# jsourati/nn-active-learning

Measured on AMD Instinct MI355X. Metric: patches/sec Fisher-scored (32^3, 2-class), higher is better.
Workload: dtype f32 (fp32 operands split into 16-bit pieces on the 16-bit MFMA, fp32 accumulate: fp16 pairs - 22-23 bits kept per operand, three products - in the conv under the head (forward + backward), in dec1's forward launch and in the other backward launches; bf16 triples - all 24 bits, exact, six products -

## Files before the change

nn-active-learning_amd/csrc/alq_internal.h:

```cpp
#pragma once
#include <hip/hip_runtime.h>

#include <cstdint>
#include <cstdio>
#include <memory>
#include <string>
#include <vector>

#include "alq.h"

namespace alq {

void set_error(const char *fmt, ...);

#define ALQ_HIP(expr)                                                                     \
    do {                                                                                  \
        hipError_t e_ = (expr);                                                           \
        if (e_ != hipSuccess) {                                                           \
            ::alq::set_error("%s:%d: %s -> %s", __FILE__, __LINE__, #expr,               \
                             hipGetErrorString(e_));                                      \
            return ALQ_EHIP;                                                              \
        }                                                                                 \
    } while (0)

// ... 190 lines not shown
    int mask_split = 0;
    long long mask_delta = 0;
    const unsigned char *mask_bits = nullptr;
    unsigned char *sign_out = nullptr;
    const unsigned *in_bits = nullptr;
    const float *in_vec = nullptr;
    float in_vec_amax = 0.f;
    const unsigned *in_vec16 = nullptr;
    unsigned *out_amax = nullptr;
    int amax_from = 0;
    const unsigned *in_amax = nullptr, *in_amax2 = nullptr;
    float in_bound = 0.f;
    const float *fc_W = nullptr;
    long long fc_F = 0;
    float *fc_part = nullptr;
    unsigned *fc_bits = nullptr;
    unsigned *flip_cnt = nullptr, *flip_list = nullptr;
    int flip_cap = 0;
    float flip_l1 = 0.f;
    bool flip_bias_nonzero = false;
};

extern unsigned long long *g_igemm2_dbg;
constexpr int ALQ_NKNOBS = 9;
extern int g_dbg_knobs[ALQ_NKNOBS];
extern int g_dcp_last_form;
extern int g_no_f16x2;
extern int g_no_fixed;
extern int g_no_xcd_order;
int igemm2_build_plan(const IgemmPlan &p1, Igemm2Plan *p2);
void igemm2_pack_weights(Igemm2Plan *p2, const std::vector<float> &Bmat);
int igemm2_launch(alq_ctx *ctx, const Igemm2Plan &plan, const View &in, const View &out, const float *bias,
                  int relu, int accumulate, int N, int prof_cls, const Igemm2Fuse *fuse);

struct Igemm3Plan {
    bool ok = false;
    bool wres = false;
    int NTW = 1;
    int wgs_per_cu = 1;
    size_t lds_bytes = 0;
    std::vector<unsigned short> h_W;
    void *d_W = nullptr;
    std::vector<unsigned short> h_W16;
    void *d_W16 = nullptr;
    int w16_exp = 0;
};
int igemm3_build_plan(const Igemm2Plan &p2, Igemm3Plan *p3);
void igemm3_pack_weights(const Igemm2Plan &p2, Igemm3Plan *p3, const std::vector<float> &Bmat);
void igemm3_pack_weights_f16(const Igemm2Plan &p2, Igemm3Plan *p3, const std::vector<float> &Bmat);
// ... 363 lines not shown
```

nn-active-learning_amd/csrc/igemm2.hip:

```cpp
#include "alq_internal.h"

#include <algorithm>
#include <cmath>
#include <cstring>

namespace alq {

typedef float f32x4 __attribute__((ext_vector_type(4)));
typedef float f32x2 __attribute__((ext_vector_type(2)));

#ifdef ALQ_STAMPS
#define STAMP(var) asm volatile("s_memtime %0\n\ts_waitcnt lgkmcnt(0)" : "=s"(var)::"memory")
#define PHASE_END(idx)                         \
    do {                                       \
        unsigned long long t_now_;             \
        STAMP(t_now_);                         \
        ph[idx] += t_now_ - t_last;            \
        t_last = t_now_;                       \
    } while (0)
#else
#define PHASE_END(idx) do {} while (0)
#endif

constexpr int I2_CBP = 12;
// ... 461 lines not shown
}

void igemm2_pack_weights(Igemm2Plan *p2, const std::vector<float> &Bmat) {
    const Igemm2Args &a = p2->a;
    const int NTW = p2->NTW, Ci = a.Ci, Co = a.Co;
    p2->h_W.assign((size_t)a.nchunks * a.ntaps * NTW * 128, 0.f);
    for (int ch = 0; ch < a.nchunks; ++ch)
        for (int tp = 0; tp < a.ntaps; ++tp)
            for (int nt = 0; nt < NTW; ++nt)
                for (int lane = 0; lane < 64; ++lane)
                    for (int s = 0; s < 2; ++s) {
                        const int c = ch * 8 + 2 * (lane >> 4) + s;
                        const int co = nt * 16 + (lane & 15);
                        if (co < Co)
                            p2->h_W[((((size_t)ch * a.ntaps + tp) * NTW + nt) * 64 + lane) * 2 + s] =
                                Bmat[((size_t)tp * Ci + c) * Co + co];
                    }
}

unsigned long long *g_igemm2_dbg = nullptr;
int g_no_f16x2 = 0;
int g_no_xcd_order = 0;
int g_no_fixed = 0;
int g_dbg_knobs[ALQ_NKNOBS] = {0, 0, 0, 0, 0, 0, 0, 0, 0};

template <int NTW, bool WRES, int GEO, bool SUMS>
static int launch2_s(alq_ctx *ctx, const Igemm2Plan &plan, const Igemm2Args &a, unsigned grid) {
    auto kfn = igemm2_kernel<NTW, WRES, GEO, SUMS>;
    if (plan.lds_bytes > 64 * 1024)
        ALQ_HIP(hipFuncSetAttribute(reinterpret_cast<const void *>(kfn), hipFuncAttributeMaxDynamicSharedMemorySize,
                                    (int)plan.lds_bytes));
    hipLaunchKernelGGL(kfn, dim3(grid), dim3(256), plan.lds_bytes, ctx->stream, a);
    ALQ_HIP(hipGetLastError());
    return ALQ_OK;
}

template <int NTW, bool WRES, int GEO>
static int launch2_t(alq_ctx *ctx, const Igemm2Plan &plan, const Igemm2Args &a, unsigned grid) {
    return (a.osumA || a.osumB) ? launch2_s<NTW, WRES, GEO, true>(ctx, plan, a, grid)
                                : launch2_s<NTW, WRES, GEO, false>(ctx, plan, a, grid);
}

int igemm2_launch(alq_ctx *ctx, const Igemm2Plan &plan, const View &in, const View &out, const float *bias, int relu,
                  int accumulate, int N, int prof_cls, const Igemm2Fuse *fuse) {
    Igemm2Args a = plan.a;
    ALQ_REQUIRE(in.C == a.Ci && in.D == a.ID && in.H == a.IH && in.W == a.IW, ALQ_EINVAL,
                "igemm2: input view does not match plan");
// ... 53 lines not shown
```

nn-active-learning_amd/csrc/kernels.hip:

```cpp
#include "alq_internal.h"

namespace alq {

typedef float f32x4 __attribute__((ext_vector_type(4)));
typedef float f32x2 __attribute__((ext_vector_type(2)));

constexpr int BOX_SLAB = 1024;

__device__ inline double wave_sum(double v) {
#pragma unroll
    for (int o = 32; o > 0; o >>= 1) v += __shfl_xor(v, o, 64);
    return v;
}
__device__ inline float wave_sumf(float v) {
#pragma unroll
    for (int o = 32; o > 0; o >>= 1) v += __shfl_xor(v, o, 64);
    return v;
}
__device__ inline double block_sum256(double v, double *sh ) {
    v = wave_sum(v);
    if ((threadIdx.x & 63) == 0) sh[threadIdx.x >> 6] = v;
    __syncthreads();
    double r = 0;
    if (threadIdx.x == 0) r = sh[0] + sh[1] + sh[2] + sh[3];
// ... 830 lines not shown
                                P.x += r[ex]; P.y += r[1 + ex]; P.z += r[2 + ex]; P.w += r[3 + ex];
                            }
                        }
                    }
#pragma unroll
                    for (int q = 0; q + 1 < KZ; ++q) s[q] = s[q + 1];
                    s[KZ - 1] = P;
                    if (pp >= KZ - 1) {
                        f32x4 box = s[0];
#pragma unroll
                        for (int q = 1; q < KZ; ++q) { box.x += s[q].x; box.y += s[q].y; box.z += s[q].z; box.w += s[q].w; }
                        const f32x4 dd = d[pp - (KZ - 1)];
                        acc += (double)dd.x * ((double)box.x + 1.0) + (double)dd.y * ((double)box.y + 1.0) +
                               (double)dd.z * ((double)box.z + 1.0) + (double)dd.w * ((double)box.w + 1.0);
                    }
                }
            }
        }
    }
    const double tot_s = block_sum256(acc, sh);
    if (threadIdx.x == 0) Spart[n * nslab_max + slab] = tot_s;
}

static size_t boxdot_tile_bytes(int zs, int H, int W, const int k[3]) {
    return (size_t)(zs + k[0] - 1) * (H + k[1] - 1) * (W + k[2] - 1) * sizeof(float);
}
static int boxdot_zs(int D, int H, int W, const int k[3]) {
    int zs = 4096 / (H * W);
    if (zs < 1) zs = 1;
    if (zs > D) zs = D;
    while (zs > 1 && boxdot_tile_bytes(zs, H, W, k) > 48 * 1024) --zs;
    return zs;
}
static size_t boxdot_lds_bytes(int D, int H, int W, const int k[3]) {
    return boxdot_tile_bytes(boxdot_zs(D, H, W, k), H, W, k);
}
static bool boxdot_use_lds(int D, int H, int W, const int k[3]) {
    return (long long)D * H * W >= 512 && boxdot_lds_bytes(D, H, W, k) <= 48 * 1024;
}

int boxdot_slabs(long long vox) { return (int)((vox + BOX_SLAB - 1) / BOX_SLAB); }
int boxdot_conv_slabs(int D, int H, int W, const int k[3]) {
    if (boxdot_use_lds(D, H, W, k)) { const int zs = boxdot_zs(D, H, W, k); return (D + zs - 1) / zs; }
    return boxdot_slabs((long long)D * H * W);
}

int k_boxdot_conv(alq_ctx *ctx, const float *dsum, const float *asum, const float *asum2, int D, int H, int W,
                  const int k[3], const int lo[3], int N, double *Spart, int nslab_max) {
    ProfScope ps(ctx, PROF_REDUCE, 0);
    if (boxdot_use_lds(D, H, W, k)) {
        const int zs = boxdot_zs(D, H, W, k);
        const bool al16 = (((uintptr_t)dsum | (uintptr_t)asum | (uintptr_t)asum2) & 15) == 0;
#define ALQ_BOXCOL(KZ, KY, KX)                                                                                        \
    if (k[0] == KZ && k[1] == KY && k[2] == KX && (W & 3) == 0 && al16) {                                              \
        hipLaunchKernelGGL((boxdot_conv_col_kernel<KZ, KY, KX>), dim3((D + zs - 1) / zs, N), dim3(256),               \
                           boxdot_lds_bytes(D, H, W, k), ctx->stream, dsum, asum, asum2, D, H, W, lo[0], lo[1], lo[2], \
                           zs, Spart, nslab_max);                                                                      \
        ALQ_LAUNCH_CHECK();                                                                                            \
        return ALQ_OK;                                                                                                 \
    }
        ALQ_BOXCOL(3, 3, 3)
        ALQ_BOXCOL(1, 3, 3)
        ALQ_BOXCOL(1, 5, 5)
#undef ALQ_BOXCOL
        hipLaunchKernelGGL(boxdot_conv_lds_kernel, dim3((D + zs - 1) / zs, N), dim3(256), boxdot_lds_bytes(D, H, W, k),
                           ctx->stream, dsum, asum, asum2, D, H, W, k[0], k[1], k[2], lo[0], lo[1], lo[2], zs, Spart,
                           nslab_max);
        ALQ_LAUNCH_CHECK();
        return ALQ_OK;
    }
    hipLaunchKernelGGL(boxdot_conv_kernel, dim3(boxdot_slabs((long long)D * H * W), N), dim3(256), 0, ctx->stream,
                       dsum, asum, asum2, D, H, W, k[0], k[1], k[2], lo[0], lo[1], lo[2], Spart, nslab_max);
    ALQ_LAUNCH_CHECK();
    return ALQ_OK;
}
// ... 40 lines not shown
                if (uz < 0 || qz >= ID) continue;
#pragma unroll
                for (int iy = 0; iy < (K + S - 1) / S; ++iy) {
                    const int ty = (py + ly) % S + iy * S, uy = py + ly - ty, qy = uy / S;
                    if (ty >= K || uy < 0 || qy >= IH) continue;
                    const float *rowp = tile + (qz * IH + qy) * IW;
#pragma unroll
                    for (int j = 0; j < 4; ++j)
#pragma unroll
                        for (int ix = 0; ix < (K + S - 1) / S; ++ix) {
                            const int tx = (px + j + lx) % S + ix * S, ux = px + j + lx - tx, qx = ux / S;
                            if (tx < K && ux >= 0 && qx < IW) box[j] += rowp[qx];
                        }
                }
            }
            acc += (double)d.x * ((double)box[0] + 1.0) + (double)d.y * ((double)box[1] + 1.0) +
                   (double)d.z * ((double)box[2] + 1.0) + (double)d.w * ((double)box[3] + 1.0);
        }
    }
    const double tot = block_sum256(acc, sh);
    if (threadIdx.x == 0) Spart[n * nslab_max + slab] = tot;
}

static bool boxdot_convT_out_ok(int ID, int IH, int IW, const int k[3], const int s[3]) {
    const long long ivox = (long long)ID * IH * IW;
    const bool shape = k[1] == 3 && k[2] == 3 && s[1] == 2 && s[2] == 2 &&
                       ((k[0] == 3 && s[0] == 2) || (k[0] == 1 && s[0] == 1 && ID == 1));
    return shape && ivox % 4 == 0 && ivox * 4 <= 48 * 1024;
}
static int boxdot_convT_zs(int ID, int IH, int IW, const int s[3]) {
    int zs = 4096 / (IH * s[1] * IW * s[2]);
    if (zs < 1) zs = 1;
    if (zs > ID * s[0]) zs = ID * s[0];
    return zs;
}
int boxdot_convT_slabs(int ID, int IH, int IW, const int k[3], const int s[3]) {
    if (boxdot_convT_out_ok(ID, IH, IW, k, s)) { const int zs = boxdot_convT_zs(ID, IH, IW, s); return (ID * s[0] + zs - 1) / zs; }
    return boxdot_slabs((long long)ID * IH * IW);
}

int k_boxdot_convT(alq_ctx *ctx, const float *dsum, const float *asum, const float *asum2, int ID, int IH, int IW,
                   const int k[3], const int s[3], const int lo[3], int N, double *Spart, int nslab_max) {
    ProfScope ps(ctx, PROF_REDUCE, 0);
    if (boxdot_convT_out_ok(ID, IH, IW, k, s)) {
        const int zs = boxdot_convT_zs(ID, IH, IW, s);
        hipLaunchKernelGGL((boxdot_convT_out_kernel<3, 2>), dim3((ID * s[0] + zs - 1) / zs, N), dim3(256),
                           (size_t)ID * IH * IW * sizeof(float), ctx->stream, dsum, asum, asum2, ID, IH, IW, k[0], lo[0],
                           lo[1], lo[2], zs, Spart, nslab_max);
        ALQ_LAUNCH_CHECK();
        return ALQ_OK;
    }
    hipLaunchKernelGGL(boxdot_convT_kernel, dim3(boxdot_slabs((long long)ID * IH * IW), N), dim3(256), 0,
                       ctx->stream, dsum, asum, asum2, ID, IH, IW, k[0], k[1], k[2], s[0], s[1], s[2], lo[0], lo[1], lo[2],
                       Spart, nslab_max);
    ALQ_LAUNCH_CHECK();
    return ALQ_OK;
}

constexpr int FC_SLICE = 8192;
int fc_small_slices(int64_t F) { return (int)((F + FC_SLICE - 1) / FC_SLICE); }

template <int NOUT, bool BITS>
__global__ __launch_bounds__(256) void fc_small_fwd_kernel(const float *act, long long F, const float *Wp,
                                                           float *partials, int nslices, unsigned *maskbits) {
    __shared__ double sh[4];
    const int slice = blockIdx.x;
    const long long n = blockIdx.y;
    const long long f0 = (long long)slice * FC_SLICE;
// ... 148 lines not shown
    for (int v = 0; v < 4; ++v) {
        a[v] = *reinterpret_cast<const f32x4 *>(wv + (w << 5) + v * 8);
        b[v] = *reinterpret_cast<const f32x4 *>(wv + (w << 5) + v * 8 + 4);
    }
    const int n0 = blockIdx.y * FC_BITS_PG, n1 = min(N, n0 + FC_BITS_PG);
    uint2 bits[FC_BITS_PG];
#pragma unroll
    for (int k = 0; k < FC_BITS_PG; ++k)
        bits[k] = n0 + k < n1 ? reinterpret_cast<const uint2 *>(maskbits)[(n0 + k) * words + w] : uint2{0u, 0u};
#pragma unroll
    for (int k = 0; k < FC_BITS_PG; ++k) {
        if (n0 + k >= n1) break;
        float out[4];
#pragma unroll
        for (int v = 0; v < 4; ++v) {
            const unsigned two = (v < 2 ? bits[k].x : bits[k].y) >> ((v & 1) * 16);
            const unsigned m = two, m2 = two >> 8;
            const float sa = ((m & 1u ? a[v].x : 0.f) + (m & 2u ? a[v].y : 0.f)) + ((m & 4u ? a[v].z : 0.f) + (m & 8u ? a[v].w : 0.f));
            const float sb = ((m2 & 1u ? b[v].x : 0.f) + (m2 & 2u ? b[v].y : 0.f)) + ((m2 & 4u ? b[v].z : 0.f) + (m2 & 8u ? b[v].w : 0.f));
            out[v] = sa + sb;
        }
        *reinterpret_cast<f32x4 *>(dsum + ((long long)(n0 + k) * F >> 3) + (w << 2)) = f32x4{out[0], out[1], out[2], out[3]};
    }
}
__global__ __launch_bounds__(64) void rowmax_u32_kernel(const unsigned *in, int len, unsigned *out) {
    const int n = blockIdx.x;
    unsigned m = 0;
    for (int k = threadIdx.x; k < len; k += 64) m = max(m, in[(long long)n * len + k]);
#pragma unroll
    for (int off = 32; off >= 1; off >>= 1) m = max(m, (unsigned)__shfl_xor((int)m, off, 64));
    if (threadIdx.x == 0) out[n] = m;
}
int k_rowmax_u32(alq_ctx *ctx, const unsigned *in, int len, int N, unsigned *out) {
    ProfScope ps(ctx, PROF_REDUCE, 0);
    hipLaunchKernelGGL(rowmax_u32_kernel, dim3(N), dim3(64), 0, ctx->stream, in, len, out);
    ALQ_LAUNCH_CHECK();
    return ALQ_OK;
}

__global__ __launch_bounds__(256) void rowmax_abs_kernel(const float *x, int N, long long K, unsigned *out) {
    const int row = blockIdx.x * 4 + (threadIdx.x >> 6), lane = threadIdx.x & 63;
    if (row >= N) return;
    const float *p = x + (size_t)row * K;
    float m = 0.f;
    if ((K & 3) == 0 && (reinterpret_cast<size_t>(x) & 15) == 0) {
        typedef float v4 __attribute__((ext_vector_type(4)));
// ... 144 lines not shown
int k_flip_fix(alq_ctx *ctx, unsigned *list, unsigned *cnt, int cap, int N, const float *inA, const float *inB, int CA, int CB,
               int D, int H, int W, int kz, int ky, int kx, int lz, int ly, int lx, const float *W32, const float *bias, int Co,
               unsigned char *bits, long long F, unsigned *overflow) {
    ProfScope ps(ctx, PROF_ELEMWISE, 0);
    ALQ_REQUIRE(F % 64 == 0, ALQ_EINVAL, "flip_fix: %lld sign bytes per patch are not whole 16-byte words", (long long)(F >> 2));
    ALQ_REQUIRE(cap >= flip_list_len(N), ALQ_EINVAL, "flip_fix: list of %d slots for %d patches", cap, N);
    if (N <= 0) return ALQ_OK;
    const long long p16 = (F >> 2) / 16;
    const unsigned segs = (unsigned)flip_segments(N);
    hipLaunchKernelGGL(flip_scan_kernel, dim3(segs), dim3(256), 0, ctx->stream, reinterpret_cast<const uint4 *>(bits), p16, cnt, list, overflow);
    if (CA + CB == 16 && kz == 3 && ky == 3 && kx == 3)
        hipLaunchKernelGGL((flip_fix_kernel<16, 3, 3, 3>), dim3(segs * 4), dim3(256), 0, ctx->stream, list, cnt, inA, inB, CA, CB, D, H, W,
                           kz, ky, kx, lz, ly, lx, W32, bias, Co, bits, F);
    else
        hipLaunchKernelGGL((flip_fix_kernel<0, 0, 0, 0>), dim3(segs * 4), dim3(256), 0, ctx->stream, list, cnt, inA, inB, CA, CB, D, H, W,
                           kz, ky, kx, lz, ly, lx, W32, bias, Co, bits, F);
    ALQ_LAUNCH_CHECK();
    return ALQ_OK;
}

int k_fc_small_dsum_bits(alq_ctx *ctx, const unsigned *maskbits, const float *wv, int64_t F, int N, float *dsum) {
    ProfScope ps(ctx, PROF_FC_SMALL, 0);
    ALQ_REQUIRE(F % 32 == 0, ALQ_EINVAL, "fc_small_dsum_bits: F %% 32");
    hipLaunchKernelGGL(fc_small_dsum_bits_kernel, dim3((unsigned)((F / 32 + 255) / 256), (unsigned)((N + FC_BITS_PG - 1) / FC_BITS_PG)),
                       dim3(256), 0, ctx->stream, maskbits, wv, (long long)F, N, dsum);
    ALQ_LAUNCH_CHECK();
    return ALQ_OK;
}

int k_fc_small_bwd(alq_ctx *ctx, const float *delta, int nout, const float *Wp, int64_t F, int N,
                   float *dact, const float *mask_act, float *dsum, int C, bool *fused) {
    ProfScope ps(ctx, PROF_FC_SMALL, 2.0 * F * nout * N);
    if (fused) *fused = false;
    if ((F & 3) == 0) {
        const int G = (dsum && C > 0 && C % 4 == 0) ? C / 4 : 0;
        const dim3 grid(grid_for((long long)N * (F >> 2)));
#define ALQ_FB(GV) \
    hipLaunchKernelGGL(fc_small_bwd_kernel<GV>, grid, dim3(256), 0, ctx->stream, delta, nout, Wp, (long long)F, N, dact, mask_act, dsum)
        if (G == 1) { ALQ_FB(1); if (fused) *fused = true; }
        else if (G == 2) { ALQ_FB(2); if (fused) *fused = true; }
        else if (G == 4) { ALQ_FB(4); if (fused) *fused = true; }
        else if (G == 8) { ALQ_FB(8); if (fused) *fused = true; }
        else hipLaunchKernelGGL(fc_small_bwd_kernel<0>, grid, dim3(256), 0, ctx->stream, delta, nout, Wp, (long long)F, N,
                                dact, (const float *)nullptr, (float *)nullptr);
#undef ALQ_FB
    } else
// ... 275 lines not shown
```

nn-active-learning_amd/csrc/model.hip:

```cpp
#include <algorithm>
#include <cmath>
#include <cstdarg>
#include <cstring>
#include <string>
#include <memory>

#include "alq_internal.h"

namespace alq {

static thread_local char g_err[1024] = "";
void set_error(const char *fmt, ...) {
    va_list ap;
    va_start(ap, fmt);
    vsnprintf(g_err, sizeof(g_err), fmt, ap);
    va_end(ap);
}

int gather_normalize_impl(alq_ctx *, const void *const *, int, int, const int64_t[3], const int64_t[3],
                          const int64_t *, int64_t, const int32_t[3], const double *, int, int, void *);
int score_entropy_impl(alq_ctx *, const float *, int64_t, double *, float *);
int synth_impl(alq_ctx *, uint64_t, int64_t, int64_t, int64_t, float *);
int gather_rows_impl(alq_ctx *, const float *, const int64_t *, int64_t, int64_t, float *);
int debug_view_copy(alq_ctx *, const View &, int, float *);
// ... 90 lines not shown
    unsigned *flip_overflow = nullptr;
    int no_flipfix = 0;
    size_t amax_tiles_len = 0;
    int in_dims[4] = {1, 1, 1, 1};
    int nclass = 0;
    int L = 0;
    std::vector<Layer> layers;
    std::vector<void *> allocs;
    float *logits = nullptr, *dlogits = nullptr, *post = nullptr;
    double *S = nullptr, *sizes = nullptr, *Apart = nullptr;
    double *Spart = nullptr;
    int *nslab = nullptr;
    int nslab_max = 1;
    float *wg_partial = nullptr;
    size_t wg_partial_len = 0;
    double *gn_partial = nullptr;
    size_t gn_partial_len = 0;
    double *ls_part = nullptr;
    std::vector<int> ls_nslab;
    int ls_nslab_max = 0;
    int last_lsum = 0;
    float *x_stage = nullptr;
    int64_t epp = 0;
    int knobs[ALQ_NKNOBS] = {0, 0, 0, 0, 0, 0, 0, 0, 0};
    int no_f16x2 = 0;
    int no_xcd_order = 0;
    int requested_batch = 0;
    int no_bound16 = 0;
    int no_fixed = 0;
    int no_presplit = 0;
    int no_signs = 0;
    int no_signs0 = 0;
    int f16_fwd_mask = -1;
    int f16_fwd_derived = 0;
    int no_f16_derived = 0;
    float *d_bound_L = nullptr, *d_bound_B = nullptr;
    int *d_bound_src = nullptr;
    int no_light_kernels = 0;
    int no_c3d = 0;
    int c3_bwd_rows = 8;
    bool last_c3 = false;
    bool last_c3_bwd = false;
    int no_e3d = 0;
    int last_e3b = 0;
    int no_d3d = 0;
    int last_d3f = 0;
    int no_f3d = 0, last_f3f = 0;
    int no_d3b = 0, last_d3b = 0;
    int no_t3d = 0;
    int last_dcp = 0;
    int last_t3f = 0, last_t3b = 0;
    bool last_f16_derived = false;
    int64_t host_pack_elems = 0;
    void *d_wscal = nullptr;
    bool hv_ready = false;
    double *hv_part = nullptr;
    double *hv_p64 = nullptr;

    template <typename T>
    int dalloc(T **p, size_t count) {
        void *q = nullptr;
        const size_t bytes = std::max<size_t>(count * sizeof(T), 256);
        if (hipMalloc(&q, bytes) != hipSuccess) {
            set_error("hipMalloc of %zu bytes failed", bytes);
            return ALQ_ENOMEM;
        }
        allocs.push_back(q);
        *p = reinterpret_cast<T *>(q);
        return ALQ_OK;
    }
};

// ... 30 lines not shown
            s.pool.push_back(pr.first);
            s.pool.push_back(pr.second);
        }
        s.pending.clear();
    }
    return ALQ_OK;
}

static int upload1(alq_model *m, IgemmPlan *p) {
    if (!p->d_W) ALQ_TRY(m->dalloc(&p->d_W, p->h_W.size()));
    ALQ_HIP(hipMemcpyAsync(p->d_W, p->h_W.data(), p->h_W.size() * sizeof(float), hipMemcpyHostToDevice,
                           m->ctx->stream));
    if (p->smallc) {
        if (!p->d_koff) ALQ_TRY(m->dalloc(&p->d_koff, p->h_koff.size()));
        ALQ_HIP(hipMemcpyAsync(p->d_koff, p->h_koff.data(), p->h_koff.size() * sizeof(int),
                               hipMemcpyHostToDevice, m->ctx->stream));
    }
    ALQ_HIP(hipStreamSynchronize(m->ctx->stream));
    std::vector<float>().swap(p->h_W);
    return ALQ_OK;
}

static bool g_use_v2 = true;
static int g_knob_override[ALQ_NKNOBS] = {-1, -1, -1, -1, -1, -1, -1, -1, -1};

static void apply_knobs(const alq_model *m) {
    for (int k = 0; k < ALQ_NKNOBS; ++k) g_dbg_knobs[k] = g_knob_override[k] >= 0 ? g_knob_override[k] : m->knobs[k];
    g_no_f16x2 = m->no_f16x2;
    g_no_xcd_order = m->no_xcd_order;
    g_no_fixed = m->no_fixed;
}

static int gemm_build(const ConvDesc &d, int max_batch, Gemm *g, const G4Geom *g4 = nullptr) {
    ALQ_TRY(igemm_build_plan(d, max_batch, &g->p1));
    if (g4 && !getenv("ALQ_DISABLE_V4")) {
        G4Geom gg = *g4;
        gg.flops_per_patch = g->p1.flops_per_patch;
        ALQ_TRY(igemm4_build_plan(gg, max_batch, &g->p4));
    }
    ALQ_TRY(igemm2_build_plan(g->p1, &g->p2));
    ALQ_TRY(direct_build_plan(g->p1, &g->pd));
    if (!g_use_v2) { g->p2.ok = false; g->pd.ok = false; }
    ALQ_TRY(igemm3_build_plan(g->p2, &g->p3));
    if (d.ID == 1 && d.IH == 1 && d.IW == 1 && d.tz.size() == 1 && d.sm == 1 && d.so == 1 && !getenv("ALQ_NO_FCGEMM"))
        ALQ_TRY(fcgemm_build_plan(d.Ci, d.Co, &g->pfc));
    if (const char *e = getenv("ALQ_DISABLE_V3")) { if (e[0] == '1') g->p3.ok = false; }
    return ALQ_OK;
// ... 898 lines not shown
        if (hipEventRecord(c->ev_fork, main) != hipSuccess || hipStreamWaitEvent(c->side, c->ev_fork, 0) != hipSuccess) {
            (void)hipGetLastError();
            return;
        }
        c->stream = c->side;
        c->side_used = true;
        on = true;
    }
    ~SideStream() { if (on) c->stream = main; }
    SideStream(const SideStream &) = delete;
    SideStream &operator=(const SideStream &) = delete;
};

static int side_join(alq_ctx *c) {
    if (!c->side || !c->side_used) return ALQ_OK;
    c->side_used = false;
    ALQ_HIP(hipEventRecord(c->ev_join, c->side));
    ALQ_HIP(hipStreamWaitEvent(c->stream, c->ev_join, 0));
    return ALQ_OK;
}

static int run_backward_main(alq_model *m, const float *d_x, int N);
static int run_backward(alq_model *m, const float *d_x, int N) {
    const int rc = run_backward_main(m, d_x, N);
    const int rj = side_join(m->ctx);
    return rc != ALQ_OK ? rc : rj;
}

static int run_backward_main(alq_model *m, const float *d_x, int N) {
    alq_ctx *ctx = m->ctx;
    const int nl = (int)m->layers.size();
    ALQ_REQUIRE(m->nclass == 2, ALQ_EUNSUPPORTED, "Fisher scoring is binary (PW_NNAL.py:766), got %d classes", m->nclass);
    ALQ_TRY(k_fill_unit_cotangent(ctx, m->dlogits, N));
    for (Layer &l : m->layers) { l.delta_ready = false; l.dsum_partial = false; l.dout_bits = nullptr; l.dout_vec = nullptr; l.dout_vec16 = nullptr; l.dout_vec16c = nullptr; l.dout_amax = nullptr; }
    m->last_c3_bwd = false;
    m->last_t3b = 0;
    const bool v4_on = !g_dbg_knobs[4] && !g_dbg_knobs[5];
    {
        for (Layer &l : m->layers) l.dout_bound = 0.f;
        m->layers[nl - 1].dout_bound = 1.f;
        for (int i = nl - 1; i >= 1; --i) {
            const Layer &ly = m->layers[i];
            double inb = ly.dout_bound;
            if (ly.spec.type == ALQ_FC)
                inb = (ly.spec.cout == 2 && ly.fc_wv_amax > 0.f && i == nl - 1) ? (double)ly.fc_wv_amax : (i < nl - 1 ? ly.bwd_l1 * ly.dout_bound : 0.0);
            else if (ly.spec.type != ALQ_POOL) inb = ly.bwd_l1 * ly.dout_bound;
            if (!(inb > 0.0) || ly.dout_bound <= 0.f) inb = 0.0;
// ... 751 lines not shown
        g_use_v2 = !(e && e[0] == '1');
        m->no_f16x2 = getenv("ALQ_NO_F16X2") != nullptr;
        m->no_xcd_order = getenv("ALQ_NO_XCD_ORDER") != nullptr;
        m->no_fixed = getenv("ALQ_NO_FIXED") != nullptr;
        m->no_bound16 = getenv("ALQ_NO_BOUND16") != nullptr;
        m->no_flipfix = getenv("ALQ_NO_FLIPFIX") != nullptr;
        m->no_presplit = getenv("ALQ_NO_PRESPLIT") != nullptr;
        m->no_c3d = getenv("ALQ_NO_C3D") != nullptr;
        m->no_light_kernels = getenv("ALQ_NO_LIGHT_KERNELS") != nullptr;
        { const char *e = getenv("ALQ_C3D_BWD_ROWS"); m->c3_bwd_rows = (e && atoi(e) == 4) ? 4 : ((e && atoi(e) == 8) ? 8 : 7); }
        m->no_signs = getenv("ALQ_NO_SIGNS") != nullptr;
        m->no_signs0 = getenv("ALQ_NO_SIGNS0") != nullptr;
        if (const char *f = getenv("ALQ_F16_FWD_MASK")) m->f16_fwd_mask = atoi(f);
        m->no_t3d = getenv("ALQ_NO_T3D") ? 1 : 0;
        m->no_e3d = getenv("ALQ_NO_E3D") ? 1 : 0;
        m->no_d3d = getenv("ALQ_NO_D3D") ? 1 : 0;
        m->no_f3d = getenv("ALQ_NO_F3D") ? 1 : 0;
        m->no_d3b = getenv("ALQ_NO_D3D_BWD") ? 1 : 0;
        {
            const char *e = getenv("ALQ_F16_DERIVED"), *n = getenv("ALQ_NO_F16_DERIVED");
            m->no_f16_derived = ((e && atoi(e) == 0) || (n && atoi(n) == 1)) ? 1 : 0;
        }
        static const char *names[ALQ_NKNOBS] = {"ALQ_DEBUG_REPEAT", "ALQ_DEBUG_FLAGS", "ALQ_NO_BWD_FUSE", "ALQ_NO_FWD_FUSE", "ALQ_NO_V3", "ALQ_NO_V4",
                                                "ALQ_NO_POOL_FIRST", "ALQ_NO_CONV_POOL", "ALQ_DCP_NARROW"};
        for (int k = 0; k < ALQ_NKNOBS; ++k) {
            const char *v = getenv(names[k]);
            if (v) m->knobs[k] = atoi(v);
        }
    }
    for (int i = 0; i < 4; ++i) m->in_dims[i] = in_dims[i];
    m->epp = (int64_t)in_dims[0] * in_dims[1] * in_dims[2] * in_dims[3];
    const int rc = build_model(m, layers, n_layers);
    if (rc != ALQ_OK) {
        alq_model_destroy(m);
        return rc;
    }
    if (const char *t = getenv("ALQ_G4_TUNE")) {
        std::string all(t);
        size_t pos = 0;
        while (pos < all.size()) {
            size_t end = all.find(';', pos);
            if (end == std::string::npos) end = all.size();
            const std::string item = all.substr(pos, end - pos);
            pos = end + 1;
            if (item.size() < 3 || (item[0] != 'f' && item[0] != 'b')) continue;
            const size_t colon = item.find(':');
            if (colon == std::string::npos) continue;
// ... 629 lines not shown
        return ALQ_OK;
    }
    if (what == 0 || what == 1) {
        const Layer &head = m->layers.back();
        ALQ_REQUIRE(!(layer_idx + 2 == (int)m->layers.size() && head.spec.type == ALQ_FC &&
                      (what == 0 ? m->last_head_fused
                                 : (m->last_call_fisher && head.fc_maskbits != nullptr && !g_dbg_knobs[4] && !g_dbg_knobs[5]))),
                    ALQ_EUNSUPPORTED, "layer %d: this tensor is not materialised in a Fisher pass (fc head fused into the layer: "
                    "create the model under ALQ_NO_FC_BITS=1 to keep it)", layer_idx);
        const View &v = what == 0 ? ly.out : ly.dout;
        if (elems_out) *elems_out = (int64_t)N * v.elems();
        return debug_view_copy(m->ctx, v, N, d_out);
    }
    ALQ_REQUIRE(ly.pidx >= 0 && (what == 2 || what == 3), ALQ_EINVAL, "layer has no channel-sum fields");
    const bool isfc = ly.spec.type == ALQ_FC;
    const int64_t e = (int64_t)N * (isfc ? 1 : (what == 2 ? ly.in.vox() : ly.out.vox()));
    if (elems_out) *elems_out = e;
    ALQ_HIP(hipMemcpyAsync(d_out, what == 2 ? ly.asum : ly.dsum, e * sizeof(float), hipMemcpyDeviceToDevice,
                           m->ctx->stream));
    return ALQ_OK;
}

int alq_model_engine_info(alq_model *m, int what) {
    ALQ_REQUIRE(m && ((what >= 0 && what <= 3) || (what >= 5 && what <= 16)), ALQ_EINVAL, "alq_model_engine_info: bad argument");
    if (what == 16) return m->last_dcp;
    if (what == 15) return m->last_lsum;
    if (what == 14) return m->host_pack_elems > 0x7fffffffll ? 0x7fffffff : (int)m->host_pack_elems;
    if (what == 13) return m->last_c3_bwd ? m->c3_bwd_rows : 0;
    if (what == 6) return m->last_f16_derived ? 1 : 0;
    if (what == 7) return m->last_t3f;
    if (what == 8) return m->last_t3b;
    if (what == 12) return m->last_f3f;
    if (what == 11) return m->last_d3b;
    if (what == 10) return m->last_d3f;
    if (what == 9) return m->last_e3b;
    ALQ_HIP(hipSetDevice(m->ctx->device));
    if (what == 0) return c3d_subnormals_ok(m->ctx);
    if (what == 1) return m->last_c3 ? 1 : 0;
    if (what == 2) return m->last_c3_bwd ? 1 : 0;
    if (what == 5) {
        if (!m->flip_overflow) return 0;
        unsigned h = 0;
        ALQ_HIP(hipMemcpyAsync(&h, m->flip_overflow, sizeof(unsigned), hipMemcpyDeviceToHost, m->ctx->stream));
        ALQ_HIP(hipStreamSynchronize(m->ctx->stream));
        return h > 0x7fffffffu ? 0x7fffffff : (int)h;
    }
    for (const Layer &ly : m->layers)
// ... 25 lines not shown
```

Baseline: 284,000.

## Add streaming variants of side-sum boxdot and fc bit-sum kernels

Adds three new kernels for the backward side-sum reductions: a 3x3x3 conv boxdot kernel that software-prefetches the next dsum column while computing the current one and uses a padded, skewed LDS row pitch; a convT boxdot kernel that stages only the input planes a slab needs, with an optional skewed layout; and an fc bit-mask dsum kernel that prefetches mask words in chunks of eight and processes several patches per block. These are meant to hide global-load latency and cut LDS bank conflicts and redundant staging in these small reductions. The old paths stay reachable through a new ALQ_SIDE_SUMS_OLD knob, and an engine-info query reports which form ran. The added complexity risks register pressure and edge-case correctness in the skewed indexing.

Result: no change. 282,800 (-0.4%).

```diff
diff --git a/nn-active-learning_amd/csrc/alq_internal.h b/nn-active-learning_amd/csrc/alq_internal.h
--- a/nn-active-learning_amd/csrc/alq_internal.h
+++ b/nn-active-learning_amd/csrc/alq_internal.h
@@ -236,9 +236,10 @@
 };
 
 extern unsigned long long *g_igemm2_dbg;
-constexpr int ALQ_NKNOBS = 9;
+constexpr int ALQ_NKNOBS = 10;
 extern int g_dbg_knobs[ALQ_NKNOBS];
 extern int g_dcp_last_form;
+extern int g_side_sums_last_form;
 extern int g_no_f16x2;
 extern int g_no_fixed;
 extern int g_no_xcd_order;
diff --git a/nn-active-learning_amd/csrc/igemm2.hip b/nn-active-learning_amd/csrc/igemm2.hip
--- a/nn-active-learning_amd/csrc/igemm2.hip
+++ b/nn-active-learning_amd/csrc/igemm2.hip
@@ -507,7 +507,7 @@
 int g_no_f16x2 = 0;
 int g_no_xcd_order = 0;
 int g_no_fixed = 0;
-int g_dbg_knobs[ALQ_NKNOBS] = {0, 0, 0, 0, 0, 0, 0, 0, 0};
+int g_dbg_knobs[ALQ_NKNOBS] = {0, 0, 0, 0, 0, 0, 0, 0, 0, 0};
 
 template <int NTW, bool WRES, int GEO, bool SUMS>
 static int launch2_s(alq_ctx *ctx, const Igemm2Plan &plan, const Igemm2Args &a, unsigned grid) {
diff --git a/nn-active-learning_amd/csrc/kernels.hip b/nn-active-learning_amd/csrc/kernels.hip
--- a/nn-active-learning_amd/csrc/kernels.hip
+++ b/nn-active-learning_amd/csrc/kernels.hip
@@ -876,6 +876,164 @@
     if (threadIdx.x == 0) Spart[n * nslab_max + slab] = tot_s;
 }
 
+static bool side_sums_old(int bit) { return (g_dbg_knobs[9] & (1 | bit)) != 0; }
+int g_side_sums_last_form = 0;
+
+template <int KZ, int KY, int KX>
+__global__ __launch_bounds__(256) void boxdot_conv_col_stream_kernel(const float *dsum, const float *asum, const float *asum2,
+                                                                     int D, int H, int W, int lz, int ly, int lx, int ZS, int PWP,
+                                                                     int SK, double *Spart, int nslab_max) {
+    extern __shared__ float tile[];
+    __shared__ double sh[4];
+    const long long n = blockIdx.y;
+    const int slab = blockIdx.x;
+    const int z0 = slab * ZS;
+    const int PH = H + KY - 1, PW = W + KX - 1, planes = ZS + KZ - 1;
+    const int vox = D * H * W;
+    const float *an = asum + n * vox;
+    const float *an2 = asum2 ? asum2 + n * vox : nullptr;
+    auto rowoff = [PWP, SK](int r) { return r * PWP + SK * (r & 1); };
+    constexpr int NR = (4 + KX) & ~1;
+    constexpr int ZR = 4;
+    const float *dn = dsum + n * vox;
+    const int cols = (H * W) >> 2;
+    const int ceff = cols < 256 ? cols : 256;
+    const int zg = 256 / ceff;
+    const int nrun = (ZS + ZR - 1) / ZR;
+    const int g = threadIdx.x / ceff;
+    int c = threadIdx.x - g * ceff, run = g;
+    const bool any = g < zg && run < nrun;
+    auto load_d = [&](int cc, int rr, f32x4 (&d)[ZR]) {
+        const int y = (cc * 4) / W, x = (cc * 4) - y * W;
+        const int zb = rr * ZR;
+#pragma unroll
+        for (int j = 0; j < ZR; ++j) {
+            const int zz = zb + j;
+            d[j] = f32x4{0.f, 0.f, 0.f, 0.f};
+            if (zz < ZS && z0 + zz < D) d[j] = *reinterpret_cast<const f32x4 *>(dn + ((z0 + zz) * H + y) * W + x);
+        }
+    };
+    f32x4 d[ZR];
+#pragma unroll
+    for (int j = 0; j < ZR; ++j) d[j] = f32x4{0.f, 0.f, 0.f, 0.f};
+    if (any) load_d(c, run, d);
+    {
+        const int W4 = W >> 2, rowq = H * W4, nq = planes * rowq;
+        int pz = threadIdx.x / rowq, rq = threadIdx.x - pz * rowq;
+        int iy = rq / W4, ixq = rq - iy * W4;
+        const int sx = 256 % W4, sy = (256 / W4) % H, sz = 256 / rowq;
+        constexpr int U = 6;
+        for (int base = threadIdx.x; base < nq; base += 256 * U) {
+            f32x4 v[U];
+            int dst[U], edge[U];
+#pragma unroll
+            for (int u = 0; u < U; ++u) {
+                dst[u] = -1;
+                edge[u] = 0;
+                v[u] = f32x4{0.f, 0.f, 0.f, 0.f};
+                if (base + u * 256 < nq) {
+                    const int iz = z0 + pz - lz;
+                    if (iz >= 0 && iz < D) {
+                        const int o = (iz * H + iy) * W + ixq * 4;
+                        v[u] = *reinterpret_cast<const f32x4 *>(an + o);
+                        if (an2) {
+                            const f32x4 w = *reinterpret_cast<const f32x4 *>(an2 + o);
+                            v[u].x += w.x; v[u].y += w.y; v[u].z += w.z; v[u].w += w.w;
+                        }
+                    }
+                    dst[u] = rowoff(pz * PH + iy + ly) + ixq * 4 + lx;
+                    edge[u] = (ixq == 0 ? 1 : 0) | (ixq == W4 - 1 ? 2 : 0);
+                }
+                ixq += sx; iy += sy; pz += sz;
+                if (ixq >= W4) { ixq -= W4; ++iy; }
+                if (iy >= H) { iy -= H; ++pz; }
+            }
+#pragma unroll
+            for (int u = 0; u < U; ++u)
+                if (dst[u] >= 0) {
+                    float *t = tile + dst[u];
+                    t[0] = v[u].x; t[1] = v[u].y; t[2] = v[u].z; t[3] = v[u].w;
+#pragma unroll
+                    for (int k = 0; k < KX - 1; ++k) {
+                        if ((edge[u] & 1) && k < lx) t[k - lx] = 0.f;
+                        if ((edge[u] & 2) && k < KX - 1 - lx) t[4 + k] = 0.f;
+                    }
+                }
+        }
+    }
+    if constexpr (KY > 1) {
+        const int tot = planes * (KY - 1) * PW;
+        for (int i = threadIdx.x; i < tot; i += 256) {
+            const int hr = i / PW, xx = i - hr * PW;
+            const int pz = hr / (KY - 1), k = hr - pz * (KY - 1);
+            tile[rowoff(pz * PH + (k < ly ? k : k + H)) + xx] = 0.f;
+        }
+    }
+    __syncthreads();
+    double acc = 0;
+    if (any) {
+        while (true) {
+            int cn = c, rn = run + zg;
+            if (rn >= nrun) { rn = g; cn = c + ceff; }
+            const bool more = cn < cols;
+            f32x4 dnx[ZR];
+#pragma unroll
+            for (int j = 0; j < ZR; ++j) dnx[j] = f32x4{0.f, 0.f, 0.f, 0.f};
+            if (more) load_d(cn, rn, dnx);
+            {
+                const int y = (c * 4) / W, x = (c * 4) - y * W;
+                const int zb = run * ZR;
+                f32x4 s[KZ];
+#pragma unroll
+                for (int q = 0; q < KZ; ++q) s[q] = f32x4{0.f, 0.f, 0.f, 0.f};
+#pragma unroll
+                for (int pp = 0; pp < ZR + KZ - 1; ++pp) {
+                    const int p = zb + pp;
+                    f32x4 P = {0.f, 0.f, 0.f, 0.f};
+                    if (p < planes) {
+#pragma unroll
+                        for (int ey = 0; ey < KY; ++ey) {
+                            const float *rowp = tile + rowoff(p * PH + (y + ey)) + x;
+                            float r[NR];
+#pragma unroll
+                            for (int j = 0; j < NR; j += 2) {
+                                const f32x2 t = *reinterpret_cast<const f32x2 *>(rowp + j);
+                                r[j] = t.x; r[j + 1] = t.y;
+                            }
+#pragma unroll
+                            for (int ex = 0; ex < KX; ++ex) {
+                                P.x += r[ex]; P.y += r[1 + ex]; P.z += r[2 + ex]; P.w += r[3 + ex];
+                            }
+                        }
+                    }
+#pragma unroll
+                    for (int q = 0; q + 1 < KZ; ++q) s[q] = s[q + 1];
+                    s[KZ - 1] = P;
+                    if (pp >= KZ - 1) {
+                        f32x4 box = s[0];
+#pragma unroll
+                        for (int q = 1; q < KZ; ++q) { box.x += s[q].x; box.y += s[q].y; box.z += s[q].z; box.w += s[q].w; }
+                        const f32x4 dd = d[pp - (KZ - 1)];
+                        acc += (double)dd.x * ((double)box.x + 1.0) + (double)dd.y * ((double)box.y + 1.0) +
+                               (double)dd.z * ((double)box.z + 1.0) + (double)dd.w * ((double)box.w + 1.0);
+                    }
+                }
+            }
+            if (!more) break;
+            c = cn; run = rn;
+#pragma unroll
+            for (int j = 0; j < ZR; ++j) d[j] = dnx[j];
+        }
+    }
+    const double tot_s = block_sum256(acc, sh);
+    if (threadIdx.x == 0) Spart[n * nslab_max + slab] = tot_s;
+}
+static void boxdot_col_pitch(int zs, int H, int W, const int k[3], int *pwp, int *sk) {
+    const int rows = (zs + k[0] - 1) * (H + k[1] - 1), PW = W + k[2] - 1;
+    *pwp = PW; *sk = 0;
+    if (W == 32 && PW + 2 <= 48 && ((size_t)rows * 48 + 2) * sizeof(float) <= 48 * 1024) { *pwp = 48; *sk = 2; }
+}
+
 static size_t boxdot_tile_bytes(int zs, int H, int W, const int k[3]) {
     return (size_t)(zs + k[0] - 1) * (H + k[1] - 1) * (W + k[2] - 1) * sizeof(float);
 }
@@ -905,6 +1063,17 @@
     if (boxdot_use_lds(D, H, W, k)) {
         const int zs = boxdot_zs(D, H, W, k);
         const bool al16 = (((uintptr_t)dsum | (uintptr_t)asum | (uintptr_t)asum2) & 15) == 0;
+        if (k[0] == 3 && k[1] == 3 && k[2] == 3 && (W & 3) == 0 && al16 && !side_sums_old(4)) {
+            int pwp, sk;
+            boxdot_col_pitch(zs, H, W, k, &pwp, &sk);
+            g_side_sums_last_form |= 1;
+            hipLaunchKernelGGL((boxdot_conv_col_stream_kernel<3, 3, 3>), dim3((D + zs - 1) / zs, N), dim3(256),
+                               ((size_t)(zs + 2) * (H + 2) * pwp + sk) * sizeof(float), ctx->stream, dsum, asum, asum2, D, H, W, lo[0],
+                               lo[1], lo[2], zs, pwp, sk, Spart, nslab_max);
+            ALQ_LAUNCH_CHECK();
+            return ALQ_OK;
+        }
+        if (k[0] == 3 && k[1] == 3 && k[2] == 3 && (W & 3) == 0 && al16) g_side_sums_last_form |= 2;
 #define ALQ_BOXCOL(KZ, KY, KX)                                                                                        \
     if (k[0] == KZ && k[1] == KY && k[2] == KX && (W & 3) == 0 && al16) {                                              \
         hipLaunchKernelGGL((boxdot_conv_col_kernel<KZ, KY, KX>), dim3((D + zs - 1) / zs, N), dim3(256),               \
@@ -991,6 +1160,99 @@
     if (threadIdx.x == 0) Spart[n * nslab_max + slab] = tot;
 }
 
+template <int K, int S>
+__global__ __launch_bounds__(256) void boxdot_convT_out_stream_kernel(const float *dsum, const float *asum, const float *asum2,
+                                                                      int ID, int IH, int IW, int kz, int lz, int ly, int lx,
+                                                                      int ZS, int SKT, double *Spart, int nslab_max) {
+    extern __shared__ float tile[];
+    __shared__ double sh[4];
+    const long long n = blockIdx.y;
+    const int slab = blockIdx.x;
+    const int sz = kz == 1 ? 1 : S;
+    const int OD = ID * sz, OH = IH * S, OW = IW * S;
+    const int ivox = ID * IH * IW;
+    const float *an = asum + n * ivox;
+    const float *an2 = asum2 ? asum2 + n * ivox : nullptr;
+    const float *dn = dsum + n * (long long)OD * OH * OW;
+    const bool al = (((uintptr_t)dn | (uintptr_t)an | (uintptr_t)an2) & 15) == 0;
+    auto ld4 = [](const float *p, bool a) {
+        return a ? *reinterpret_cast<const f32x4 *>(p) : f32x4{p[0], p[1], p[2], p[3]};
+    };
+    const int z0 = slab * ZS;
+    const int z1 = min(OD, z0 + ZS);
+    const int OW4 = OW >> 2, ncol = OH * OW4;
+    const int ceff = ncol < 256 ? ncol : 256, zg = 256 / ceff, g = threadIdx.x / ceff;
+    int c = threadIdx.x - g * ceff, pz = z0 + g;
+    const bool any = g < zg && pz < z1;
+    auto load_d = [&](int cc, int zz) {
+        const int py = cc / OW4, px = (cc - py * OW4) * 4;
+        return ld4(dn + ((long long)zz * OH + py) * OW + px, al);
+    };
+    f32x4 d = {0.f, 0.f, 0.f, 0.f};
+    if (any) d = load_d(c, pz);
+    int qlo = 0, np = ID;
+    const int plane = IH * IW;
+    if ((plane & 3) == 0) {
+        const int lo_u = z0 + lz - (kz - 1);
+        qlo = lo_u <= 0 ? 0 : (lo_u + sz - 1) / sz;
+        const int qhi = min(ID - 1, (z1 - 1 + lz) / sz);
+        np = qhi - qlo + 1;
+    }
+    {
+        const int cnt = np * plane;
+        const float *a1 = an + (long long)qlo * plane;
+        const float *a2 = an2 ? an2 + (long long)qlo * plane : nullptr;
+        for (int i = threadIdx.x * 4; i < cnt; i += 1024) {
+            f32x4 v = ld4(a1 + i, al);
+            if (a2) {
+                const f32x4 w = ld4(a2 + i, al);
+                v.x += w.x; v.y += w.y; v.z += w.z; v.w += w.w;
+            }
+            float *t = tile + i + (SKT ? (i / IW) >> 1 : 0);
+            t[0] = v.x; t[1] = v.y; t[2] = v.z; t[3] = v.w;
+        }
+    }
+    __syncthreads();
+    double acc = 0;
+    if (any) {
+        while (true) {
+            int cn = c, zn = pz + zg;
+            if (zn >= z1) { zn = z0 + g; cn = c + ceff; }
+            const bool more = cn < ncol;
+            f32x4 dnx = {0.f, 0.f, 0.f, 0.f};
+            if (more) dnx = load_d(cn, zn);
+            {
+                const int py = c / OW4, px = (c - py * OW4) * 4;
+                float box[4] = {0.f, 0.f, 0.f, 0.f};
+                for (int tz = (pz + lz) % sz; tz < kz; tz += sz) {
+                    const int uz = pz + lz - tz, qz = uz / sz;
+                    if (uz < 0 || qz >= ID) continue;
+#pragma unroll
+                    for (int iy = 0; iy < (K + S - 1) / S; ++iy) {
+                        const int ty = (py + ly) % S + iy * S, uy = py + ly - ty, qy = uy / S;
+                        if (ty >= K || uy < 0 || qy >= IH) continue;
+                        const int r = (qz - qlo) * IH + qy;
+                        const float *rowp = tile + r * IW + (SKT ? r >> 1 : 0);
+#pragma unroll
+                        for (int j = 0; j < 4; ++j)
+#pragma unroll
+                            for (int ix = 0; ix < (K + S - 1) / S; ++ix) {
+                                const int tx = (px + j + lx) % S + ix * S, ux = px + j + lx - tx, qx = ux / S;
+                                if (tx < K && ux >= 0 && qx < IW) box[j] += rowp[qx];
+                            }
+                    }
+                }
+                acc += (double)d.x * ((double)box[0] + 1.0) + (double)d.y * ((double)box[1] + 1.0) +
+                       (double)d.z * ((double)box[2] + 1.0) + (double)d.w * ((double)box[3] + 1.0);
+            }
+            if (!more) break;
+            c = cn; pz = zn; d = dnx;
+        }
+    }
+    const double tot = block_sum256(acc, sh);
+    if (threadIdx.x == 0) Spart[n * nslab_max + slab] = tot;
+}
+
 static bool boxdot_convT_out_ok(int ID, int IH, int IW, const int k[3], const int s[3]) {
     const long long ivox = (long long)ID * IH * IW;
     const bool shape = k[1] == 3 && k[2] == 3 && s[1] == 2 && s[2] == 2 &&
@@ -1013,6 +1275,17 @@
     ProfScope ps(ctx, PROF_REDUCE, 0);
     if (boxdot_convT_out_ok(ID, IH, IW, k, s)) {
         const int zs = boxdot_convT_zs(ID, IH, IW, s);
+        if (!side_sums_old(8)) {
+            g_side_sums_last_form |= 1;
+            const size_t skewed = ((size_t)ID * IH * IW + (size_t)ID * IH / 2 + 1) * sizeof(float);
+            const int skt = ((IW & 3) == 0 && skewed <= 48 * 1024) ? 1 : 0;
+            hipLaunchKernelGGL((boxdot_convT_out_stream_kernel<3, 2>), dim3((ID * s[0] + zs - 1) / zs, N), dim3(256),
+                               skt ? skewed : (size_t)ID * IH * IW * sizeof(float), ctx->stream, dsum, asum, asum2, ID, IH, IW, k[0], lo[0],
+                               lo[1], lo[2], zs, skt, Spart, nslab_max);
+            ALQ_LAUNCH_CHECK();
+            return ALQ_OK;
+        }
+        g_side_sums_last_form |= 2;
         hipLaunchKernelGGL((boxdot_convT_out_kernel<3, 2>), dim3((ID * s[0] + zs - 1) / zs, N), dim3(256),
                            (size_t)ID * IH * IW * sizeof(float), ctx->stream, dsum, asum, asum2, ID, IH, IW, k[0], lo[0],
                            lo[1], lo[2], zs, Spart, nslab_max);
@@ -1207,6 +1480,50 @@
         }
         *reinterpret_cast<f32x4 *>(dsum + ((long long)(n0 + k) * F >> 3) + (w << 2)) = f32x4{out[0], out[1], out[2], out[3]};
     }
+}
+constexpr int FC_BITS_CH = 8;
+__device__ __forceinline__ f32x4 fc_bits_sums(const uint2 bits, const f32x4 (&a)[4], const f32x4 (&b)[4]) {
+    float out[4];
+#pragma unroll
+    for (int v = 0; v < 4; ++v) {
+        const unsigned two = (v < 2 ? bits.x : bits.y) >> ((v & 1) * 16);
+        const unsigned m = two, m2 = two >> 8;
+        const float sa = ((m & 1u ? a[v].x : 0.f) + (m & 2u ? a[v].y : 0.f)) + ((m & 4u ? a[v].z : 0.f) + (m & 8u ? a[v].w : 0.f));
+        const float sb = ((m2 & 1u ? b[v].x : 0.f) + (m2 & 2u ? b[v].y : 0.f)) + ((m2 & 4u ? b[v].z : 0.f) + (m2 & 8u ? b[v].w : 0.f));
+        out[v] = sa + sb;
+    }
+    return f32x4{out[0], out[1], out[2], out[3]};
+}
+__global__ __launch_bounds__(256) void fc_small_dsum_stream_kernel(const unsigned *maskbits, const float *wv, long long F, int N,
+                                                                   int ppg, float *dsum) {
+    const long long words = F >> 5;
+    const long long w = blockIdx.x * (long long)blockDim.x + threadIdx.x;
+    if (w >= words) return;
+    f32x4 a[4], b[4];
+#pragma unroll
+    for (int v = 0; v < 4; ++v) {
+        a[v] = *reinterpret_cast<const f32x4 *>(wv + (w << 5) + v * 8);
+        b[v] = *reinterpret_cast<const f32x4 *>(wv + (w << 5) + v * 8 + 4);
+    }
+    const int n0 = blockIdx.y * ppg, n1 = min(N, n0 + ppg);
+    const uint2 *mb = reinterpret_cast<const uint2 *>(maskbits) + w;
+    float *dp = dsum + (w << 2);
+    const long long dstride = F >> 3;
+    uint2 cur[FC_BITS_CH], nxt[FC_BITS_CH];
+#pragma unroll
+    for (int k = 0; k < FC_BITS_CH; ++k) cur[k] = mb[(long long)min(n0 + k, n1 - 1) * words];
+    int n = n0;
+    for (; n + FC_BITS_CH <= n1; n += FC_BITS_CH) {
+#pragma unroll
+        for (int k = 0; k < FC_BITS_CH; ++k) nxt[k] = mb[(long long)min(n + FC_BITS_CH + k, n1 - 1) * words];
+#pragma unroll
+        for (int k = 0; k < FC_BITS_CH; ++k) *reinterpret_cast<f32x4 *>(dp + (long long)(n + k) * dstride) = fc_bits_sums(cur[k], a, b);
+#pragma unroll
+        for (int k = 0; k < FC_BITS_CH; ++k) cur[k] = nxt[k];
+    }
+#pragma unroll
+    for (int k = 0; k < FC_BITS_CH - 1; ++k)
+        if (n + k < n1) *reinterpret_cast<f32x4 *>(dp + (long long)(n + k) * dstride) = fc_bits_sums(cur[k], a, b);
 }
 __global__ __launch_bounds__(64) void rowmax_u32_kernel(const unsigned *in, int len, unsigned *out) {
     const int n = blockIdx.x;
@@ -1397,6 +1714,17 @@
 int k_fc_small_dsum_bits(alq_ctx *ctx, const unsigned *maskbits, const float *wv, int64_t F, int N, float *dsum) {
     ProfScope ps(ctx, PROF_FC_SMALL, 0);
     ALQ_REQUIRE(F % 32 == 0, ALQ_EINVAL, "fc_small_dsum_bits: F %% 32");
+    if (!side_sums_old(2) && N > 0) {
+        const unsigned gx = (unsigned)((F / 32 + 255) / 256);
+        const int gy_want = (int)std::max(1u, 1024u / gx);
+        const int ppg = std::max((N + gy_want - 1) / gy_want, FC_BITS_CH);
+        g_side_sums_last_form |= 1;
+        hipLaunchKernelGGL(fc_small_dsum_stream_kernel, dim3(gx, (unsigned)((N + ppg - 1) / ppg)), dim3(256), 0, ctx->stream, maskbits, wv,
+                           (long long)F, N, ppg, dsum);
+        ALQ_LAUNCH_CHECK();
+        return ALQ_OK;
+    }
+    g_side_sums_last_form |= 2;
     hipLaunchKernelGGL(fc_small_dsum_bits_kernel, dim3((unsigned)((F / 32 + 255) / 256), (unsigned)((N + FC_BITS_PG - 1) / FC_BITS_PG)),
                        dim3(256), 0, ctx->stream, maskbits, wv, (long long)F, N, dsum);
     ALQ_LAUNCH_CHECK();
diff --git a/nn-active-learning_amd/csrc/model.hip b/nn-active-learning_amd/csrc/model.hip
--- a/nn-active-learning_amd/csrc/model.hip
+++ b/nn-active-learning_amd/csrc/model.hip
@@ -136,7 +136,7 @@
     int last_lsum = 0;
     float *x_stage = nullptr;
     int64_t epp = 0;
-    int knobs[ALQ_NKNOBS] = {0, 0, 0, 0, 0, 0, 0, 0, 0};
+    int knobs[ALQ_NKNOBS] = {0, 0, 0, 0, 0, 0, 0, 0, 0, 0};
     int no_f16x2 = 0;
     int no_xcd_order = 0;
     int requested_batch = 0;
@@ -162,6 +162,7 @@
     int no_f3d = 0, last_f3f = 0;
     int no_d3b = 0, last_d3b = 0;
     int no_t3d = 0;
+    int last_side_sums = 0;
     int last_dcp = 0;
     int last_t3f = 0, last_t3b = 0;
     bool last_f16_derived = false;
@@ -238,7 +239,7 @@
 }
 
 static bool g_use_v2 = true;
-static int g_knob_override[ALQ_NKNOBS] = {-1, -1, -1, -1, -1, -1, -1, -1, -1};
+static int g_knob_override[ALQ_NKNOBS] = {-1, -1, -1, -1, -1, -1, -1, -1, -1, -1};
 
 static void apply_knobs(const alq_model *m) {
     for (int k = 0; k < ALQ_NKNOBS; ++k) g_dbg_knobs[k] = g_knob_override[k] >= 0 ? g_knob_override[k] : m->knobs[k];
@@ -1183,7 +1184,9 @@
 
 static int run_backward_main(alq_model *m, const float *d_x, int N);
 static int run_backward(alq_model *m, const float *d_x, int N) {
+    g_side_sums_last_form = 0;
     const int rc = run_backward_main(m, d_x, N);
+    m->last_side_sums = g_side_sums_last_form;
     const int rj = side_join(m->ctx);
     return rc != ALQ_OK ? rc : rj;
 }
@@ -1981,7 +1984,7 @@
             m->no_f16_derived = ((e && atoi(e) == 0) || (n && atoi(n) == 1)) ? 1 : 0;
         }
         static const char *names[ALQ_NKNOBS] = {"ALQ_DEBUG_REPEAT", "ALQ_DEBUG_FLAGS", "ALQ_NO_BWD_FUSE", "ALQ_NO_FWD_FUSE", "ALQ_NO_V3", "ALQ_NO_V4",
-                                                "ALQ_NO_POOL_FIRST", "ALQ_NO_CONV_POOL", "ALQ_DCP_NARROW"};
+                                                "ALQ_NO_POOL_FIRST", "ALQ_NO_CONV_POOL", "ALQ_DCP_NARROW", "ALQ_SIDE_SUMS_OLD"};
         for (int k = 0; k < ALQ_NKNOBS; ++k) {
             const char *v = getenv(names[k]);
             if (v) m->knobs[k] = atoi(v);
@@ -2657,7 +2660,8 @@
 }
 
 int alq_model_engine_info(alq_model *m, int what) {
-    ALQ_REQUIRE(m && ((what >= 0 && what <= 3) || (what >= 5 && what <= 16)), ALQ_EINVAL, "alq_model_engine_info: bad argument");
+    ALQ_REQUIRE(m && ((what >= 0 && what <= 3) || (what >= 5 && what <= 17)), ALQ_EINVAL, "alq_model_engine_info: bad argument");
+    if (what == 17) return m->last_side_sums;
     if (what == 16) return m->last_dcp;
     if (what == 15) return m->last_lsum;
     if (what == 14) return m->host_pack_elems > 0x7fffffffll ? 0x7fffffff : (int)m->host_pack_elems;
```
